# Many98/Crop2Seg

Hardware: AMD Instinct MI355X
Metric: train patches/sec (Tx10x128x128) U-TAE (higher is better)
Workload: dtype f32

## Files before the change

### crop2seg_amd/csrc/loss.hip

```cpp
#include "common.h"

namespace {

constexpr int MAXK = C2S_MAX_CLASSES;
constexpr int LOSS_BLOCKS = 512;

__device__ __forceinline__ bool valid_target(long long t, int K, long long ignore_index) {
    return !(t == ignore_index || t < 0 || t >= K);
}

__device__ __forceinline__ size_t pixel_offset(long e, int K, int HW) {
    const int pix = (int)(e % HW), b = (int)(e / HW);
    return (size_t)b * K * HW + pix;
}

__device__ __forceinline__ void zero_row(float* __restrict__ gp, int K, int HW) {
    for (int k = 0; k < K; ++k) gp[(size_t)k * HW] = 0.f;
}

template <bool FAST>
__device__ __forceinline__ void softmax_stats(const float* __restrict__ lp, int K, int HW, float& mx, float& s) {
    mx = lp[0];
    for (int k = 1; k < K; ++k) mx = fmaxf(mx, lp[(size_t)k * HW]);
    s = 0.f;
    for (int k = 0; k < K; ++k) s += FAST ? __expf(lp[(size_t)k * HW] - mx) : expf(lp[(size_t)k * HW] - mx);
}

template <int N>
__device__ __forceinline__ void block_partials(float (&v)[N], float* __restrict__ part) {
    __shared__ float red[4][N];
#pragma unroll
    for (int j = 0; j < N; ++j) v[j] = wave_sum(v[j]);
    if ((threadIdx.x & 63) == 0)
        for (int j = 0; j < N; ++j) red[threadIdx.x >> 6][j] = v[j];
    __syncthreads();
    if (threadIdx.x == 0)
        for (int j = 0; j < N; ++j) part[blockIdx.x * N + j] = (red[0][j] + red[1][j]) + (red[2][j] + red[3][j]);
}

template <int N>
__device__ __forceinline__ void sum_partials(const float* __restrict__ part, int blocks, double (&acc)[N]) {
    for (int i = 0; i < blocks; ++i) {
#pragma unroll
        for (int j = 0; j < N; ++j) acc[j] += part[i * N + j];
    }
}
__device__ __forceinline__ void store_loss(float* __restrict__ loss, float l, int accumulate) {
    *loss = accumulate ? *loss + l : l;
}

__global__ __launch_bounds__(256) void ce_fwd_kernel(const float* __restrict__ logits, const int64_t* __restrict__ target,
                                                     const float* __restrict__ cw, float* __restrict__ part, int B, int K,
                                                     int HW, float eps, long long ignore_index) {
    const long total = (long)B * HW;
    float num = 0.f, den = 0.f, bad = 0.f;
    for (long e = blockIdx.x * (long)blockDim.x + threadIdx.x; e < total; e += (long)gridDim.x * blockDim.x) {
        const long long yy = target[e];
        if (!valid_target(yy, K, ignore_index)) { bad += yy != ignore_index ? 1.f : 0.f; continue; }
        const int y = (int)yy;
        const float* lp = logits + pixel_offset(e, K, HW);
        float mx, s;
        softmax_stats<true>(lp, K, HW, mx, s);
        const float w = cw[y];
        const float lse = mx + __logf(s);
        float li = w * (lse - lp[(size_t)y * HW]);
        if (eps > 0.f) {
            float sm = 0.f;
            for (int k = 0; k < K; ++k) sm += cw[k] * (lse - lp[(size_t)k * HW]);
            li = (1.f - eps) * li + (eps / (float)K) * sm;
        }
        num += li;
        den += w;
    }
    float v[3] = {num, den, bad};
    block_partials(v, part);
}

__global__ void ce_finalize_kernel(const float* __restrict__ part, float* __restrict__ tot, float* __restrict__ loss,
                                   int blocks) {
    if (threadIdx.x != 0 || blockIdx.x != 0) return;
    double a[3] = {};
    sum_partials(part, blocks, a);
    tot[0] = (float)a[0]; tot[1] = (float)a[1]; tot[2] = (float)a[2];
    store_loss(loss, (float)(a[0] / a[1]), 0);
}

__global__ __launch_bounds__(256) void ce_bwd_kernel(const float* __restrict__ logits, const int64_t* __restrict__ target,
                                                     const float* __restrict__ cw, const float* __restrict__ tot,
                                                     float* __restrict__ glogits, int B, int K, int HW, float eps,
                                                     long long ignore_index) {
    const long total = (long)B * HW;
    const float inv_den = 1.f / tot[1];
    float wsum = 0.f;
    if (eps > 0.f)
        for (int k = 0; k < K; ++k) wsum += cw[k];
    for (long e = blockIdx.x * (long)blockDim.x + threadIdx.x; e < total; e += (long)gridDim.x * blockDim.x) {
        const float* lp = logits + pixel_offset(e, K, HW);
        float* gp = glogits + pixel_offset(e, K, HW);
        const long long yy = target[e];
        if (!valid_target(yy, K, ignore_index)) { zero_row(gp, K, HW); continue; }
        const int y = (int)yy;
        float mx, s;
        softmax_stats<true>(lp, K, HW, mx, s);
        const float w = cw[y] * inv_den, inv_s = 1.f / s;
        if (eps > 0.f) {
            const float a = (1.f - eps) * w, c = eps / (float)K * inv_den;
            for (int k = 0; k < K; ++k) {
                const float pk = __expf(lp[(size_t)k * HW] - mx) * inv_s;
                gp[(size_t)k * HW] = a * (pk - (k == y ? 1.f : 0.f)) + c * (wsum * pk - cw[k]);
            }
        } else {
            for (int k = 0; k < K; ++k)
                gp[(size_t)k * HW] = w * (__expf(lp[(size_t)k * HW] - mx) * inv_s - (k == y ? 1.f : 0.f));
        }
    }
}

__global__ __launch_bounds__(256) void focal_fwd_kernel(const float* __restrict__ logits, const int64_t* __restrict__ target,
                                                        const float* __restrict__ class_w, float* __restrict__ part, int B, int K,
                                                        int HW, float gamma, long long ignore_index) {
    const long total = (long)B * HW;
    float num = 0.f, cnt = 0.f, wsum = 0.f;
    for (long e = blockIdx.x * 256L + threadIdx.x; e < total; e += (long)gridDim.x * 256) {
        const long long t = target[e];
        if (!valid_target(t, K, ignore_index)) continue;
        const float* lp = logits + pixel_offset(e, K, HW);
        float mx, s;
        softmax_stats<false>(lp, K, HW, mx, s);
        const float logpt = lp[(size_t)t * HW] - mx - logf(s);
        const float pt = expf(logpt);
        num += -powf(1.f - pt, gamma) * logpt;
        cnt += 1.f;
        wsum += class_w ? class_w[t] : 1.f;
    }
    float v[3] = {num, cnt, wsum};
    block_partials(v, part);
}

__global__ void focal_finalize_kernel(const float* __restrict__ part, float* __restrict__ tot, float* __restrict__ loss,
                                      int blocks, int weighted, int size_average, int accumulate) {
    if (threadIdx.x != 0 || blockIdx.x != 0) return;
    double a[3] = {};
    sum_partials(part, blocks, a);
    const double num = a[0], cnt = a[1], wsum = a[2];
    const double scale = weighted ? (size_average ? wsum / (cnt * cnt) : wsum) : (size_average ? 1.0 / cnt : 1.0);
    tot[0] = (float)num; tot[1] = (float)cnt; tot[2] = (float)scale;
    store_loss(loss, (float)(num * scale), accumulate);
}

__global__ __launch_bounds__(256) void focal_bwd_kernel(const float* __restrict__ logits, const int64_t* __restrict__ target,
                                                        const float* __restrict__ tot, float* __restrict__ glogits, int B,
                                                        int K, int HW, float gamma, long long ignore_index) {
    const long total = (long)B * HW;
    const float inv_n = tot[2];
    for (long e = blockIdx.x * 256L + threadIdx.x; e < total; e += (long)gridDim.x * 256) {
        const float* lp = logits + pixel_offset(e, K, HW);
        float* gp = glogits + pixel_offset(e, K, HW);
        const long long t = target[e];
        if (!valid_target(t, K, ignore_index)) { zero_row(gp, K, HW); continue; }
        float mx, s;
        softmax_stats<false>(lp, K, HW, mx, s);
        const float inv_s = 1.f / s;
        const float logpt = lp[(size_t)t * HW] - mx - logf(s);
        const float pt = expf(logpt);
        const float om = 1.f - pt;
        const bool at_limit = gamma < 1.f && (gamma == 0.f || om <= 0.f);
        const float om_gm1 = at_limit ? 0.f : powf(om, gamma - 1.f);
        const float coef = (gamma * om_gm1 * pt * logpt - powf(om, gamma)) * inv_n;
        for (int k = 0; k < K; ++k) {
            const float pk = expf(lp[(size_t)k * HW] - mx) * inv_s;
            gp[(size_t)k * HW] = coef * ((k == t ? 1.f : 0.f) - pk);
        }
    }
}

__global__ __launch_bounds__(256) void smooth_ce_kernel(const float* __restrict__ logits, const int64_t* __restrict__ target,
// ... 21 lines not shown
        if (r < H - 1) { const long long v = target[e + W]; if (v >= 0 && v < K) mask |= 1u << (int)v; }
        if (x > 0) { const long long v = target[e - 1]; if (v >= 0 && v < K) mask |= 1u << (int)v; }
        if (x < W - 1) { const long long v = target[e + 1]; if (v >= 0 && v < K) mask |= 1u << (int)v; }
        const float nd = (float)__popc(mask);
        const float exp_small = eps * ((float)K - nd);
        const float exp_large = (1.f - exp_small) / nd;
        const bool is_bg = bg != nullptr && t == bg_index;
        float mx, s;
        softmax_stats<false>(lp, K, HW, mx, s);
        const float lse = mx + logf(s);
        const float inv_s = 1.f / s;
        float loss = 0.f, wsum = 0.f;
        for (int k = 0; k < K; ++k) {
            const float tk = is_bg ? bg[k] : (((mask >> k) & 1u) ? exp_large : eps);
            const float wt = (class_w ? class_w[k] : 1.f) * tk;
            loss -= wt * (lp[(size_t)k * HW] - lse);
            wsum += wt;
        }
        num += loss;
        if (pixel_loss) pixel_loss[e] = loss;
        if (gp) {
            for (int k = 0; k < K; ++k) {
                const float tk = is_bg ? bg[k] : (((mask >> k) & 1u) ? exp_large : eps);
                const float wt = (class_w ? class_w[k] : 1.f) * tk;
                const float pk = expf(lp[(size_t)k * HW] - mx) * inv_s;
                gp[(size_t)k * HW] = (pk * wsum - wt) * inv_n;
            }
        }
    }
    float v[2] = {num, bad};
    block_partials(v, part);
}

__global__ void smooth_ce_finalize_kernel(const float* __restrict__ part, float* __restrict__ tot, float* __restrict__ loss,
                                          int blocks, double npix, int accumulate) {
    if (threadIdx.x != 0 || blockIdx.x != 0) return;
    double a[2] = {};
    sum_partials(part, blocks, a);
    tot[0] = (float)a[0]; tot[1] = (float)a[1];
    store_loss(loss, (float)(a[0] / npix), accumulate);
}

constexpr int NCOUNT = 2 * MAXK + 1;

inline size_t recall_ws_floats(long n) { return (size_t)n + LOSS_BLOCKS + (2 * NCOUNT + 1) + MAXK + 2; }

__global__ void recall_zero_kernel(unsigned long long* __restrict__ cnt) {
    for (int i = threadIdx.x; i < NCOUNT; i += blockDim.x) cnt[i] = 0ull;
}

__device__ __forceinline__ void load_pixel(const float* __restrict__ lp, int K, int HW, float (&v)[MAXK]) {
#pragma unroll
    for (int k = 0; k < MAXK; ++k)
        if (k < K) v[k] = lp[(size_t)k * HW];
}

__global__ __launch_bounds__(256) void recall_count_kernel(const float* __restrict__ logits, const int64_t* __restrict__ target,
                                                           float* __restrict__ nll, unsigned long long* __restrict__ cnt, int B,
                                                           int K, int HW, long long ignore_index) {
    __shared__ unsigned int h[NCOUNT];
    for (int i = threadIdx.x; i < NCOUNT; i += 256) h[i] = 0;
    __syncthreads();
    const long total = (long)B * HW;
    for (long e = blockIdx.x * 256L + threadIdx.x; e < total; e += (long)gridDim.x * 256) {
        const long long t = target[e];
        if (!valid_target(t, K, ignore_index)) {
            if (t != ignore_index) atomicAdd(&h[2 * MAXK], 1u);
            nll[e] = 0.f;
            continue;
        }
        float v[MAXK];
// ... 19 lines not shown
    for (int i = threadIdx.x; i < NCOUNT; i += 256)
        if (h[i]) atomicAdd(cnt + i, (unsigned long long)h[i]);
}

__global__ void recall_weights_kernel(const unsigned long long* __restrict__ cnt, float* __restrict__ w, float* __restrict__ tot,
                                      float* __restrict__ weights_out, long long* __restrict__ counts_out, int K) {
    const int k = threadIdx.x;
    if (k < K) {
        const unsigned long long gt = cnt[k], fn = cnt[MAXK + k];
        const float wk = (float)((double)(fn > 0 ? fn : 1ull) / (double)(gt > 0 ? gt : 1ull));
        w[k] = wk;
        if (weights_out) weights_out[k] = wk;
        if (counts_out) { counts_out[k] = (long long)gt; counts_out[K + k] = (long long)fn; }
    }
    if (k == 0) tot[1] = (float)cnt[2 * MAXK];
}

__global__ __launch_bounds__(256) void recall_loss_kernel(const float* __restrict__ nll, const int64_t* __restrict__ target,
                                                          const float* __restrict__ w, float* __restrict__ part, long total,
                                                          int K, long long ignore_index) {
    __shared__ float ws[MAXK];
    if (threadIdx.x < K) ws[threadIdx.x] = w[threadIdx.x];
    __syncthreads();
    float num = 0.f;
    for (long e = blockIdx.x * 256L + threadIdx.x; e < total; e += (long)gridDim.x * 256) {
        const long long t = target[e];
        if (!valid_target(t, K, ignore_index)) continue;
        num += ws[(int)t] * nll[e];
    }
    float v[1] = {num};
    block_partials(v, part);
}

__global__ void recall_finalize_kernel(const float* __restrict__ part, float* __restrict__ tot, float* __restrict__ loss,
                                       int blocks, double npix, int accumulate) {
    if (threadIdx.x != 0 || blockIdx.x != 0) return;
    double a[1] = {};
    sum_partials(part, blocks, a);
    tot[0] = (float)a[0];
    store_loss(loss, (float)(a[0] / npix), accumulate);
}

__global__ __launch_bounds__(256) void recall_bwd_kernel(const float* __restrict__ logits, const int64_t* __restrict__ target,
                                                         const float* __restrict__ w, float* __restrict__ glogits, int B, int K,
                                                         int HW, long long ignore_index, float inv_n) {
    __shared__ float ws[MAXK];
    if (threadIdx.x < K) ws[threadIdx.x] = w[threadIdx.x];
    __syncthreads();
    const long total = (long)B * HW;
    for (long e = blockIdx.x * 256L + threadIdx.x; e < total; e += (long)gridDim.x * 256) {
        float* gp = glogits + pixel_offset(e, K, HW);
        const long long t = target[e];
        if (!valid_target(t, K, ignore_index)) { zero_row(gp, K, HW); continue; }
        float v[MAXK];
        load_pixel(logits + pixel_offset(e, K, HW), K, HW, v);
        float mx = v[0];
#pragma unroll
        for (int k = 1; k < MAXK; ++k)
            if (k < K) mx = fmaxf(mx, v[k]);
        float s = 0.f;
#pragma unroll
        for (int k = 0; k < MAXK; ++k)
            if (k < K) { v[k] = expf(v[k] - mx); s += v[k]; }
        const float inv_s = 1.f / s, c = ws[(int)t] * inv_n;
#pragma unroll
        for (int k = 0; k < MAXK; ++k)
            if (k < K) gp[(size_t)k * HW] = c * (v[k] * inv_s - (k == (int)t ? 1.f : 0.f));
    }
}

}

extern "C" size_t c2s_cross_entropy_workspace_floats(int, int) { return 3 * LOSS_BLOCKS + 3; }

extern "C" int c2s_cross_entropy(const float* logits, const int64_t* target, const float* class_w, float* loss,
                                 float* glogits, int B, int K, int HW, float label_smoothing, long long ignore_index,
                                 float* workspace, size_t ws_floats, void* stream) {
    C2S_REQUIRE(logits && target && class_w && loss && workspace, "cross_entropy: null pointer");
    C2S_REQUIRE(ws_floats >= 3 * LOSS_BLOCKS + 3 && B > 0 && K > 0 && HW > 0, "cross_entropy: bad args");
    C2S_REQUIRE(label_smoothing >= 0.f && label_smoothing <= 1.f, "cross_entropy: label_smoothing must be in [0, 1]");
    hipStream_t st = (hipStream_t)stream;
    const int blocks = grid_for((long)B * HW, LOSS_BLOCKS);
    float* tot = workspace + 3 * LOSS_BLOCKS;
    hipLaunchKernelGGL(ce_fwd_kernel, dim3(blocks), dim3(256), 0, st, logits, target, class_w, workspace, B, K, HW,
                       label_smoothing, ignore_index);
    C2S_CHECK_LAUNCH("ce_fwd");
    hipLaunchKernelGGL(ce_finalize_kernel, dim3(1), dim3(64), 0, st, workspace, tot, loss, blocks);
    C2S_CHECK_LAUNCH("ce_finalize");
    if (glogits != nullptr) {
        hipLaunchKernelGGL(ce_bwd_kernel, dim3(blocks), dim3(256), 0, st, logits, target, class_w, tot, glogits, B, K, HW,
                           label_smoothing, ignore_index);
        C2S_CHECK_LAUNCH("ce_bwd");
    }
    return C2S_OK;
}

extern "C" size_t c2s_focal_ce_workspace_floats(void) { return 3 * LOSS_BLOCKS + 4; }

extern "C" int c2s_focal_ce_ex(const float* logits, const long long* target, const float* class_w, float* loss, float* glogits,
                               int B, int K, int HW, float gamma, long long ignore_index, int size_average, int accumulate_loss,
                               float* workspace, size_t ws_floats, void* stream) {
    C2S_REQUIRE(logits && target && loss && workspace, "focal_ce: null pointer");
    C2S_REQUIRE(B > 0 && K > 0 && HW > 0 && gamma >= 0.f, "focal_ce: bad args");
    C2S_REQUIRE(ws_floats >= c2s_focal_ce_workspace_floats(), "focal_ce: workspace too small");
    hipStream_t st = (hipStream_t)stream;
    const int blocks = grid_for((long)B * HW, LOSS_BLOCKS);
    float* tot = workspace + 3 * LOSS_BLOCKS;
    hipLaunchKernelGGL(focal_fwd_kernel, dim3(blocks), dim3(256), 0, st, logits, (const int64_t*)target, class_w, workspace, B, K,
                       HW, gamma, ignore_index);
    C2S_CHECK_LAUNCH("focal_fwd");
    hipLaunchKernelGGL(focal_finalize_kernel, dim3(1), dim3(64), 0, st, workspace, tot, loss, blocks, class_w != nullptr ? 1 : 0,
                       size_average, accumulate_loss);
    C2S_CHECK_LAUNCH("focal_finalize");
    if (glogits) {
        hipLaunchKernelGGL(focal_bwd_kernel, dim3(grid_for((long)B * HW, 2048)), dim3(256), 0, st, logits, (const int64_t*)target, tot,
                           glogits, B, K, HW, gamma, ignore_index);
        C2S_CHECK_LAUNCH("focal_bwd");
    }
    return C2S_OK;
}

extern "C" int c2s_focal_ce(const float* logits, const long long* target, float* loss, float* glogits, int B, int K, int HW,
                            float gamma, long long ignore_index, int accumulate_loss, float* workspace, size_t ws_floats,
                            void* stream) {
    return c2s_focal_ce_ex(logits, target, nullptr, loss, glogits, B, K, HW, gamma, ignore_index, 1, accumulate_loss, workspace,
                           ws_floats, stream);
}

extern "C" size_t c2s_smooth_ce_workspace_floats(void) { return 2 * LOSS_BLOCKS + 2; }

extern "C" int c2s_smooth_ce_ex(const float* logits, const long long* target, const float* class_w, const float* bg_distrib,
                                float* loss, float* glogits, float* pixel_loss, int B, int K, int H, int W, float label_smoothing,
                                long long bg_index, int reduction, int accumulate_loss, float* workspace, size_t ws_floats,
                                void* stream) {
    C2S_REQUIRE(logits && target && loss && workspace, "smooth_ce: null pointer");
    C2S_REQUIRE(B > 0 && H > 0 && W > 0 && K >= 1 && K <= MAXK, "smooth_ce: 1 <= K <= 32 classes");
    C2S_REQUIRE(label_smoothing >= 0.f && label_smoothing <= 1.f, "smooth_ce: label_smoothing outside [0, 1]");
    C2S_REQUIRE(reduction >= 0 && reduction <= 2 && (reduction != 2 || pixel_loss != nullptr), "smooth_ce: reduction 0 mean / 1 sum / 2 none (needs pixel_loss)");
    C2S_REQUIRE(ws_floats >= c2s_smooth_ce_workspace_floats(), "smooth_ce: workspace too small");
    hipStream_t st = (hipStream_t)stream;
    const int blocks = grid_for((long)B * H * W, LOSS_BLOCKS);
    float* tot = workspace + 2 * LOSS_BLOCKS;
    const double npix = reduction == 0 ? (double)B * H * W : 1.0;
    hipLaunchKernelGGL(smooth_ce_kernel, dim3(blocks), dim3(256), 0, st, logits, (const int64_t*)target, class_w, bg_distrib,
                       workspace, glogits, pixel_loss, B, K, H, W, label_smoothing, bg_index, (float)(1.0 / npix));
    C2S_CHECK_LAUNCH("smooth_ce");
    hipLaunchKernelGGL(smooth_ce_finalize_kernel, dim3(1), dim3(64), 0, st, workspace, tot, loss, blocks, npix, accumulate_loss);
    C2S_CHECK_LAUNCH("smooth_ce_finalize");
    return C2S_OK;
}

extern "C" int c2s_smooth_ce(const float* logits, const long long* target, const float* class_w, const float* bg_distrib,
                             float* loss, float* glogits, int B, int K, int H, int W, float label_smoothing,
                             long long bg_index, int accumulate_loss, float* workspace, size_t ws_floats, void* stream) {
    return c2s_smooth_ce_ex(logits, target, class_w, bg_distrib, loss, glogits, nullptr, B, K, H, W, label_smoothing, bg_index, 0,
                            accumulate_loss, workspace, ws_floats, stream);
}

extern "C" size_t c2s_recall_ce_workspace_floats(int B, int HW) {
    return (B > 0 && HW > 0) ? recall_ws_floats((long)B * HW) : recall_ws_floats(0);
}

extern "C" int c2s_recall_ce(const float* logits, const long long* target, float* loss, float* glogits, float* weights_out,
                             long long* counts_out, int B, int K, int HW, long long ignore_index, int accumulate_loss,
                             float* workspace, size_t ws_floats, void* stream) {
    C2S_REQUIRE(K >= 1 && K <= MAXK, "recall_ce: 1 <= K <= 32 classes (got %d)", K);
    C2S_REQUIRE(logits && target && loss && workspace, "recall_ce: null pointer");
    C2S_REQUIRE(B > 0 && HW > 0, "recall_ce: bad args");
    C2S_REQUIRE(ws_floats >= c2s_recall_ce_workspace_floats(B, HW), "recall_ce: workspace too small");
    hipStream_t st = (hipStream_t)stream;
    const long n = (long)B * HW;
    const int blocks = grid_for(n, LOSS_BLOCKS);
    float* nll = workspace;
    float* part = workspace + n;
    float* cnt_f = part + LOSS_BLOCKS;
    if (((uintptr_t)cnt_f & 7) != 0) ++cnt_f;
    unsigned long long* cnt = (unsigned long long*)cnt_f;
    float* w = part + LOSS_BLOCKS + (2 * NCOUNT + 1);
    float* tot = w + MAXK;
    hipLaunchKernelGGL(recall_zero_kernel, dim3(1), dim3(128), 0, st, cnt);
    C2S_CHECK_LAUNCH("recall_zero");
    hipLaunchKernelGGL(recall_count_kernel, dim3(blocks), dim3(256), 0, st, logits, (const int64_t*)target, nll, cnt, B, K, HW,
                       ignore_index);
    C2S_CHECK_LAUNCH("recall_count");
    hipLaunchKernelGGL(recall_weights_kernel, dim3(1), dim3(64), 0, st, cnt, w, tot, weights_out, counts_out, K);
    C2S_CHECK_LAUNCH("recall_weights");
    hipLaunchKernelGGL(recall_loss_kernel, dim3(blocks), dim3(256), 0, st, nll, (const int64_t*)target, w, part, n, K,
                       ignore_index);
    C2S_CHECK_LAUNCH("recall_loss");
    hipLaunchKernelGGL(recall_finalize_kernel, dim3(1), dim3(64), 0, st, part, tot, loss, blocks, (double)n, accumulate_loss);
    C2S_CHECK_LAUNCH("recall_finalize");
    if (glogits != nullptr) {
        hipLaunchKernelGGL(recall_bwd_kernel, dim3(blocks), dim3(256), 0, st, logits, (const int64_t*)target, w, glogits, B, K, HW,
                           ignore_index, (float)(1.0 / (double)n));
        C2S_CHECK_LAUNCH("recall_bwd");
    }
    return C2S_OK;
}
```

### crop2seg_amd/csrc/ltae.hip

```cpp
#include "common.h"
#include "ltae_drop.h"
#include "ltae_long.h"

#define C2S_AS1 __attribute__((address_space(1)))
#define C2S_AS3 __attribute__((address_space(3)))

namespace {

#ifdef C2S_LT_STAMP
__device__ unsigned long long lt_stamps[4096 * 8];
__device__ unsigned long long lt_stamps_bwd[4096 * 8];
#define LT_STAMP(k) do { if (threadIdx.x == 0 && blockIdx.x < 4096) lt_stamps[blockIdx.x * 8 + (k)] = __builtin_amdgcn_s_memtime(); } while (0)
#define LT_STAMP_B(k) do { if (threadIdx.x == 0 && blockIdx.x < 4096) lt_stamps_bwd[blockIdx.x * 8 + (k)] = __builtin_amdgcn_s_memtime(); } while (0)
#else
#define LT_STAMP(k)
#define LT_STAMP_B(k)
#endif

constexpr int NH = 16;
constexpr int DV = 16;

struct LtaeParams {
    const float* x; const float* gamma; const float* beta; const float* U; const float* s0;
    const float* Wc; const float* bc; const float* pe; const int* valid;
// ... 936 lines not shown
        __syncthreads();
        if constexpr (GX) {
            m1 = group_total(m1, red) * inv_n;
            m2 = group_total(m2, red + 256) * inv_n;
        }
        const float dgs = (dg.x + dg.y) + (dg.z + dg.w), dbs = (db.x + db.y) + (db.z + db.w);
        if constexpr (NTH > 1) {
            red[512 + (sth * C + sc_) * 2] = dgs;
            red[512 + (sth * C + sc_) * 2 + 1] = dbs;
            __syncthreads();
            if (sth == 0) {
                float a = 0.f, bsum = 0.f;
#pragma unroll
                for (int k = 0; k < NTH; ++k) { a += red[512 + (k * C + sc_) * 2]; bsum += red[512 + (k * C + sc_) * 2 + 1]; }
                p.part_gb[((size_t)tile * C + sc_) * 2] = a;
                p.part_gb[((size_t)tile * C + sc_) * 2 + 1] = bsum;
            }
        } else {
            p.part_gb[((size_t)tile * C + sc_) * 2] = dgs;
            p.part_gb[((size_t)tile * C + sc_) * 2 + 1] = dbs;
        }
        if constexpr (!GX) return;
        const f32x4 rstd = *reinterpret_cast<const f32x4*>(STl + g * 8 + 4);
        for (int t = sth; t < T; t += NTH) {
            f32x4* gp = reinterpret_cast<f32x4*>(gxc + (size_t)t * C * HW);
            const f32x4 xn = *reinterpret_cast<const f32x4*>(xs + (size_t)(t * CP + sc_) * 4);
            *gp = rstd * (*gp - m1 - xn * m2);
        }
    }
}

constexpr int RR_SLICES = 32;
template <typename TI, typename TO>
__global__ __launch_bounds__(1024) void reduce_rows_kernel(const TI* __restrict__ part, TO* __restrict__ out, TO* __restrict__ out1,
                                                           int count, int K, int slices, int rows_per_slice) {
    __shared__ double sh[16][64];
    const int lane = threadIdx.x & 63, w = threadIdx.x >> 6;
    const int k = blockIdx.x * 64 + lane;
    const int grp = blockIdx.y / slices, sl = blockIdx.y - grp * slices;
    const int r0 = sl * rows_per_slice;
    const int n = count - r0 < rows_per_slice ? count - r0 : rows_per_slice;
    const bool live = k < K;
    const TI* src = part + ((size_t)grp * count + r0) * K + (live ? k : 0);
    double s = 0.0;
    for (int i0 = w; i0 < n; i0 += 256) {
        TI v[16];
#pragma unroll
        for (int u = 0; u < 16; ++u) {
            const int i = i0 + 16 * u;
            v[u] = (live && i < n) ? src[(size_t)i * K] : TI(0);
        }
#pragma unroll
        for (int u = 0; u < 16; ++u) s += (double)v[u];
    }
    sh[w][lane] = s;
    __syncthreads();
    if (w == 0 && live) {
        double t = 0.0;
#pragma unroll
        for (int ww = 0; ww < 16; ++ww) t += sh[ww][lane];
        if (out1 != nullptr) ((k & 1) ? out1 : out)[k >> 1] = (TO)t;
        else out[(size_t)blockIdx.y * K + k] = (TO)t;
    }
}

void reduce_rows(const float* part, float* out, int groups, int count, int K, double* tmp, hipStream_t st, float* out1 = nullptr) {
    const int kb = (K + 63) / 64;
    if (count <= 512 || tmp == nullptr) {
        hipLaunchKernelGGL((reduce_rows_kernel<float, float>), dim3(kb, groups), dim3(1024), 0, st, part, out, out1, count, K, 1, count);
    } else {
        const int rps_min = (count + RR_SLICES - 1) / RR_SLICES;
        const int rps = rps_min > 256 ? rps_min : 256;
        const int slices = (count + rps - 1) / rps;
        hipLaunchKernelGGL((reduce_rows_kernel<float, double>), dim3(kb, groups * slices), dim3(1024), 0, st, part, tmp, (double*)nullptr,
                           count, K, slices, rps);
        hipLaunchKernelGGL((reduce_rows_kernel<double, float>), dim3(kb, groups), dim3(1024), 0, st, (const double*)tmp, out, out1,
                           slices, K, 1, slices);
    }
}

__global__ __launch_bounds__(64) void sum_over_pixels_kernel(const float* __restrict__ V, float* __restrict__ out, int B,
                                                             int rows, int HW) {
    const int row = blockIdx.x, lane = threadIdx.x;
    float s = 0.f;
    for (int b = 0; b < B; ++b) {
        const float* v = V + ((size_t)b * rows + row) * HW;
        for (int i = lane; i < HW; i += 64) s += v[i];
    }
    s = wave_sum(s);
    if (lane == 0) out[row] = s;
}

template <int NH = 16, int DV = 16>
__global__ __launch_bounds__(256) void gwc_kernel(const float* __restrict__ ge, const float* __restrict__ Z,
                                                  float* __restrict__ gWc, int B, int C, int HW) {
    const int h = blockIdx.x / C, c = blockIdx.x % C;
    const int q = threadIdx.x & 15;
#pragma unroll
    for (int j0 = 0; j0 < DV; j0 += 16) {
        const int j = j0 + (threadIdx.x >> 4);
        if (DV < 16 && j >= DV) break;
        float s = 0.f;
        for (int b = 0; b < B; ++b) {
            const float* z = Z + (((size_t)b * NH + h) * C + c) * HW;
            const float* g = ge + ((size_t)b * NH * DV + h * DV + j) * HW;
            for (int i = q; i < HW; i += 16) s += g[i] * z[i];
        }
        s += __shfl_xor(s, 1, 64); s += __shfl_xor(s, 2, 64); s += __shfl_xor(s, 4, 64); s += __shfl_xor(s, 8, 64);
        if (q == 0) gWc[(size_t)(h * DV + j) * C + c] = s;
    }
}

typedef float f32x4v __attribute__((ext_vector_type(4)));
constexpr int GW_PITCH = 68;
__global__ __launch_bounds__(256) void gwc_mfma_kernel(const float* __restrict__ ge, const float* __restrict__ Z,
                                                       float* __restrict__ part, int B, int HW, int tiles_per_slice) {
    constexpr int C = 64;
    __shared__ float tl[(DV + C) * GW_PITCH];
    const int h = blockIdx.x, slice = blockIdx.y;
    const int tid = threadIdx.x, lane = tid & 63, w = tid >> 6;
    const int tiles_per_b = HW / 64;
    const int ntiles = B * tiles_per_b;
    f32x4v acc = {0.f, 0.f, 0.f, 0.f};
    for (int tile = slice * tiles_per_slice; tile < (slice + 1) * tiles_per_slice && tile < ntiles; ++tile) {
        const int b = tile / tiles_per_b, pix0 = (tile % tiles_per_b) * 64;
        __syncthreads();
#pragma unroll
        for (int i = 0; i < 5; ++i) {
            const int e = tid + i * 256;
            const int row = e >> 4, q = e & 15;
            const float* src = row < DV ? ge + ((size_t)b * NH * DV + h * DV + row) * HW
                                        : Z + (((size_t)b * NH + h) * C + (row - DV)) * HW;
            *reinterpret_cast<f32x4v*>(tl + row * GW_PITCH + 4 * q) = *reinterpret_cast<const f32x4v*>(src + pix0 + 4 * q);
        }
        __syncthreads();
        const float* ap = tl + (lane & 15) * GW_PITCH + (lane >> 4);
        const float* bp = tl + (DV + w * 16 + (lane & 15)) * GW_PITCH + (lane >> 4);
#pragma unroll
        for (int ks = 0; ks < 16; ++ks) acc = __builtin_amdgcn_mfma_f32_16x16x4f32(ap[4 * ks], bp[4 * ks], acc, 0, 0, 0);
// ... 140 lines not shown
    }
    acc = wave_sum(acc);
    if (lane == 0) {
        const float vb = rsq * qv * S;
        gbk[hd] = acc_bk ? gbk[hd] + vb : vb;
        const float vq = rsq * (acc + bk[hd] * S);
        gQ[hd] = acc_q ? gQ[hd] + vq : vq;
    }
}

__global__ void pixel_gn_fwd_kernel(const float* __restrict__ x, const float* __restrict__ gamma,
                                    const float* __restrict__ beta, float* __restrict__ y, float* __restrict__ stats,
                                    int B, int C, int HW, int groups, float eps) {
    const long total = (long)B * groups * HW;
    const long e = blockIdx.x * (long)blockDim.x + threadIdx.x;
    if (e >= total) return;
    const int pix = (int)(e % HW);
    const long bg = e / HW;
    const int g = (int)(bg % groups), b = (int)(bg / groups);
    const int cpg = C / groups;
    const float* xp = x + ((size_t)b * C + g * cpg) * HW + pix;
    float s = 0.f;
    for (int c = 0; c < cpg; ++c) s += xp[(size_t)c * HW];
    const float mean = s / cpg;
    float m2 = 0.f;
    for (int c = 0; c < cpg; ++c) { const float d = xp[(size_t)c * HW] - mean; m2 += d * d; }
    const float rstd = rsqrtf(m2 / cpg + eps);
    stats[e * 2] = mean; stats[e * 2 + 1] = rstd;
    float* yp = y + ((size_t)b * C + g * cpg) * HW + pix;
    for (int c = 0; c < cpg; ++c)
        yp[(size_t)c * HW] = (xp[(size_t)c * HW] - mean) * rstd * gamma[g * cpg + c] + beta[g * cpg + c];
}

__global__ __launch_bounds__(64) void pixel_gn_bwd_kernel(const float* __restrict__ x, const float* __restrict__ gy,
                                                          const float* __restrict__ gamma, const float* __restrict__ stats,
                                                          float* __restrict__ gx, float* __restrict__ part, int B, int C,
                                                          int HW, int groups, int chunks) {
    const int lane = threadIdx.x;
    const int chunk = blockIdx.x % chunks;
    const int bg = blockIdx.x / chunks;
    const int g = bg % groups, b = bg / groups;
    const int cpg = C / groups;
    const int len = (HW + chunks - 1) / chunks;
    const int beg = chunk * len, end = (beg + len) < HW ? (beg + len) : HW;
    float dg[16], db[16];
#pragma unroll
    for (int c = 0; c < 16; ++c) { dg[c] = 0.f; db[c] = 0.f; }
    for (int pix = beg + lane; pix < end; pix += 64) {
        const long e = ((long)b * groups + g) * HW + pix;
        const float mean = stats[e * 2], rstd = stats[e * 2 + 1];
        const float* xp = x + ((size_t)b * C + g * cpg) * HW + pix;
        const float* gp = gy + ((size_t)b * C + g * cpg) * HW + pix;
        float m1 = 0.f, m2 = 0.f;
#pragma unroll
        for (int c = 0; c < 16; ++c)
            if (c < cpg) {
                const float xn = (xp[(size_t)c * HW] - mean) * rstd;
                const float gg = gp[(size_t)c * HW];
                dg[c] += gg * xn; db[c] += gg;
                const float dxn = gg * gamma[g * cpg + c];
                m1 += dxn; m2 += dxn * xn;
            }
        m1 /= cpg; m2 /= cpg;
        float* gxp = gx + ((size_t)b * C + g * cpg) * HW + pix;
#pragma unroll
        for (int c = 0; c < 16; ++c)
            if (c < cpg) {
                const float xn = (xp[(size_t)c * HW] - mean) * rstd;
                gxp[(size_t)c * HW] = rstd * (gp[(size_t)c * HW] * gamma[g * cpg + c] - m1 - xn * m2);
            }
    }
#pragma unroll
    for (int c = 0; c < 16; ++c)
        if (c < cpg) {
            const float a = wave_sum(dg[c]), bb = wave_sum(db[c]);
            if (lane == 0) {
                const size_t o = (((size_t)b * chunks + chunk) * C + g * cpg + c) * 2;
                part[o] = a; part[o + 1] = bb;
            }
        }
}

__global__ void dropout_nchw_kernel(const float* __restrict__ x, float* __restrict__ y, int B, int C, int HW, float p,
                                    uint64_t seed0, const uint64_t* __restrict__ seed_dev, const float* __restrict__ keep) {
    const uint64_t seed = seed0 + (seed_dev != nullptr ? *seed_dev * 0x9E3779B97F4A7C15ull : 0ull);
    const long total = (long)B * C * HW;
    const float inv = 1.f / (1.f - p);
    for (long e = blockIdx.x * (long)blockDim.x + threadIdx.x; e < total; e += (long)gridDim.x * blockDim.x) {
        const int pix = (int)(e % HW);
        const long bc = e / HW;
        const int c = (int)(bc % C), b = (int)(bc / C);
        const long idx = ((long)b * HW + pix) * C + c;
        const bool k = keep != nullptr ? keep[idx] != 0.f : c2s_uniform(seed, (uint64_t)idx) >= p;
        y[e] = k ? x[e] * inv : 0.f;
    }
}

__global__ void ltae_prep_kernel(const float* __restrict__ U, const float* __restrict__ gamma, const float* __restrict__ beta,
                                 float* __restrict__ Ut, float* __restrict__ cU, int C) {
    const int tid = threadIdx.x;
    for (int e = tid; e < C * NH; e += blockDim.x) {
        const int c = e / NH, h = e % NH;
        Ut[e] = U[h * C + c] * gamma[c];
    }
    if (tid < NH) {
        float s = 0.f;
        for (int c = 0; c < C; ++c) s = fmaf(U[tid * C + c], beta[c], s);
        cU[tid] = s;
    }
}


template <int CPG>
// ... 2083 lines not shown
            else hipLaunchKernelGGL((ltae_lds_bwd_kernel<256, false>), tiles, dim3(256), lb, st, p, sb);
        }
        C2S_CHECK_LAUNCH("ltae_lds_bwd");
        break;
    }
    case BWD_TILE8:
        launch_tile_bwd_heads(d, p, tiles, st);
        C2S_CHECK_LAUNCH("ltae_bwd_heads");
        break;
    }
    switch (pl.dx) {
    case DX_GX64: {
        const dim3 grid(d->B * (d->HW / 64));
        if (gx != nullptr) hipLaunchKernelGGL(ltae_stream_bwd_gx64_kernel<true>, grid, dim3(1024), GX_FLOATS * sizeof(float) + 8192, st, p, sb);
        else hipLaunchKernelGGL(ltae_stream_bwd_gx64_kernel<false>, grid, dim3(1024), GX_FLOATS * sizeof(float) + 8192, st, p, sb);
        C2S_CHECK_LAUNCH("ltae_stream_bwd_gx");
        break;
    }
    case DX_GX4: {
        const size_t lds2 = ((size_t)NH * d->C * SPT + 2 * SCH * 4 * SPT * 4) * sizeof(float);
        hipLaunchKernelGGL(ltae_stream_bwd_gx_kernel<4>, tiles, dim3(1024), lds2, st, p, sb);
        C2S_CHECK_LAUNCH("ltae_stream_bwd_gx");
        break;
    }
    case DX_TILE8:
        if (gx != nullptr) launch_tile_bwd_gx<true>(d, p, tiles, st);
        else launch_tile_bwd_gx<false>(d, p, tiles, st);
        C2S_CHECK_LAUNCH("ltae_bwd_gx");
        break;
    case DX_NONE: case DX_FUSED:
        break;
    }
    const int nh = d->n_head, dm = d->d_model;
    reduce_rows(p.part_s0, gs0, d->B, (d->HW + pl.px - 1) / pl.px, d->T * nh, rtmp, st);
    C2S_CHECK_LAUNCH("ltae_reduce_s0");
    reduce_rows(p.part_bc, gbc, 1, (int)pl.tiles, dm, rtmp, st);
    C2S_CHECK_LAUNCH("ltae_reduce_bc");
    if (call.gb) {
        reduce_rows(p.part_gb, ggamma, 1, pl.gb_tiles, 2 * d->C, rtmp, st, gbeta);
        C2S_CHECK_LAUNCH("ltae_reduce_gb");
    }
    if (pl.gU_rows) reduce_rows(part_U, gU, 1, (int)pl.tiles, nh * d->C, rtmp, st);
    else hipLaunchKernelGGL(sum_over_pixels_kernel, dim3(nh * d->C), dim3(64), 0, st, p.V, gU, d->B, nh * d->C, d->HW);
    C2S_CHECK_LAUNCH("ltae_gU");
    switch (pl.gwc) {
    case GWC_MFMA: {
        float* part_wc = workspace + ws.part_wc;
        const int tps = (d->B * (d->HW / 64) + pl.wc_slices - 1) / pl.wc_slices;
        hipLaunchKernelGGL(gwc_mfma_kernel, dim3(NH, pl.wc_slices), dim3(256), 0, st, g_emb, p.Z, part_wc, d->B, d->HW, tps);
        C2S_CHECK_LAUNCH("ltae_gWc_mfma");
        reduce_rows(part_wc, gWc, 1, pl.wc_slices, NH * DV * d->C, nullptr, st);
        C2S_CHECK_LAUNCH("ltae_gWc_reduce");
        break;
    }
    case GWC_DIRECT: {
#define F(H, D) hipLaunchKernelGGL((gwc_kernel<H, D>), dim3(nh * d->C), dim3(256), 0, st, g_emb, p.Z, gWc, d->B, d->C, d->HW)
        C2S_LTAE_HEADS(d, F)
#undef F
        C2S_CHECK_LAUNCH("ltae_gWc");
        break;
    }
    case GWC_ZERO:
        hipMemsetAsync(gWc, 0, (size_t)dm * d->C * sizeof(float), st);
        break;
    }
    return C2S_OK;
}

extern "C" int c2s_positional_table_ex(const long long* dates, float* pe, long n, float period, int d_v, void* stream) {
    C2S_REQUIRE(dates && pe && n > 0 && period > 0.f && d_v > 0, "positional_table: bad args");
    hipLaunchKernelGGL(positional_table_kernel, dim3(cdiv(n * d_v, 256)), dim3(256), 0, (hipStream_t)stream, dates, pe, n, period, d_v);
    C2S_CHECK_LAUNCH("positional_table");
    return C2S_OK;
}

extern "C" int c2s_positional_table(const long long* dates, float* pe, long n, float period, void* stream) {
    return c2s_positional_table_ex(dates, pe, n, period, DV, stream);
// ... 72 lines not shown

extern "C" int c2s_ltae_fold_bwd(const float* Q, const float* Wk, const float* bk, const float* Wc, const float* bc,
                                 const float* pe, const float* qwk, const float* gU, const float* gs0,
                                 const float* gWc_attn, const float* gbc_attn, float* gQ, float* gWk, float* gbk,
                                 float* gWc, float* gbc, int BT, int C, int acc_mask, float* workspace, size_t ws_floats,
                                 void* stream) {
    return c2s_ltae_fold_bwd_ex(Q, Wk, bk, Wc, bc, pe, qwk, gU, gs0, gWc_attn, gbc_attn, gQ, gWk, gbk, gWc, gbc, BT, C, NH, 4,
                                NH * DV, acc_mask, workspace, ws_floats, stream);
}

extern "C" int c2s_pixel_gn_fwd(const float* x, const float* gamma, const float* beta, float* y, float* stats, int B,
                                int C, int HW, int groups, float eps, void* stream) {
    C2S_REQUIRE(x && gamma && beta && y && stats && groups > 0 && C % groups == 0 && C / groups <= 16, "pixel_gn_fwd: bad args");
    const long total = (long)B * groups * HW;
    hipLaunchKernelGGL(pixel_gn_fwd_kernel, dim3(cdiv(total, 256)), dim3(256), 0, (hipStream_t)stream, x, gamma, beta, y,
                       stats, B, C, HW, groups, eps);
    C2S_CHECK_LAUNCH("pixel_gn_fwd");
    return C2S_OK;
}

extern "C" size_t c2s_pixel_gn_bwd_workspace_floats(int B, int C, int HW) {
    const int chunks = cdiv(HW, 256);
    return (size_t)B * chunks * C * 2 + 2 * (size_t)C;
}

extern "C" int c2s_pixel_gn_bwd(const float* x, const float* gy, const float* gamma, const float* stats, float* gx,
                                float* dgamma, float* dbeta, int B, int C, int HW, int groups, float* workspace,
                                size_t ws_floats, void* stream) {
    C2S_REQUIRE(x && gy && gamma && stats && gx && dgamma && dbeta && workspace, "pixel_gn_bwd: null pointer");
    C2S_REQUIRE(groups > 0 && C % groups == 0 && C / groups <= 16, "pixel_gn_bwd: bad groups");
    C2S_REQUIRE(ws_floats >= c2s_pixel_gn_bwd_workspace_floats(B, C, HW), "pixel_gn_bwd: workspace too small");
    const int chunks = cdiv(HW, 256);
    hipStream_t st = (hipStream_t)stream;
    hipLaunchKernelGGL(pixel_gn_bwd_kernel, dim3(B * groups * chunks), dim3(64), 0, st, x, gy, gamma, stats, gx, workspace,
                       B, C, HW, groups, chunks);
    C2S_CHECK_LAUNCH("pixel_gn_bwd");
    reduce_rows(workspace, dgamma, 1, B * chunks, 2 * C, nullptr, st, dbeta);
    C2S_CHECK_LAUNCH("pixel_gn_reduce");
    return C2S_OK;
}

extern "C" int c2s_dropout_nchw(const float* x, float* y, int B, int C, int HW, float p, uint64_t seed,
                                const uint64_t* seed_dev, const float* keep,
                                void* stream) {
    C2S_REQUIRE(x && y && p >= 0.f && p < 1.f, "dropout: bad args");
    const long total = (long)B * C * HW;
    const int blocks = (int)((total + 255) / 256 > 4096 ? 4096 : (total + 255) / 256);
    hipLaunchKernelGGL(dropout_nchw_kernel, dim3(blocks), dim3(256), 0, (hipStream_t)stream, x, y, B, C, HW, p, seed, seed_dev, keep);
    C2S_CHECK_LAUNCH("dropout");
    return C2S_OK;
}
```

Measured before the change: 385.2.

## Fuse loss finalize into backward, batch L-TAE reductions, widen GN backward and gWc

```diff
diff --git a/crop2seg_amd/csrc/loss.hip b/crop2seg_amd/csrc/loss.hip
--- a/crop2seg_amd/csrc/loss.hip
+++ b/crop2seg_amd/csrc/loss.hip
@@ -40,10 +40,23 @@
 
 template <int N>
 __device__ __forceinline__ void sum_partials(const float* __restrict__ part, int blocks, double (&acc)[N]) {
-    for (int i = 0; i < blocks; ++i) {
+    __shared__ double tot_red[4][N];
+#pragma unroll
+    for (int j = 0; j < N; ++j) acc[j] = 0.0;
+    for (int i = threadIdx.x; i < blocks; i += 256) {
 #pragma unroll
         for (int j = 0; j < N; ++j) acc[j] += part[i * N + j];
     }
+#pragma unroll
+    for (int j = 0; j < N; ++j) {
+#pragma unroll
+        for (int o = 32; o > 0; o >>= 1) acc[j] += __shfl_xor(acc[j], o, 64);
+    }
+    if ((threadIdx.x & 63) == 0)
+        for (int j = 0; j < N; ++j) tot_red[threadIdx.x >> 6][j] = acc[j];
+    __syncthreads();
+#pragma unroll
+    for (int j = 0; j < N; ++j) acc[j] = (tot_red[0][j] + tot_red[1][j]) + (tot_red[2][j] + tot_red[3][j]);
 }
 __device__ __forceinline__ void store_loss(float* __restrict__ loss, float l, int accumulate) {
     *loss = accumulate ? *loss + l : l;
@@ -76,21 +89,29 @@
     block_partials(v, part);
 }
 
-__global__ void ce_finalize_kernel(const float* __restrict__ part, float* __restrict__ tot, float* __restrict__ loss,
-                                   int blocks) {
-    if (threadIdx.x != 0 || blockIdx.x != 0) return;
-    double a[3] = {};
+__device__ __forceinline__ float ce_totals(const float* __restrict__ part, int blocks, float* __restrict__ tot,
+                                           float* __restrict__ loss) {
+    double a[3];
     sum_partials(part, blocks, a);
-    tot[0] = (float)a[0]; tot[1] = (float)a[1]; tot[2] = (float)a[2];
-    store_loss(loss, (float)(a[0] / a[1]), 0);
+    if (blockIdx.x == 0 && threadIdx.x == 0) {
+        tot[0] = (float)a[0]; tot[1] = (float)a[1]; tot[2] = (float)a[2];
+        store_loss(loss, (float)(a[0] / a[1]), 0);
+    }
+    return (float)a[1];
+}
+
+__global__ __launch_bounds__(256) void ce_finalize_kernel(const float* __restrict__ part, float* __restrict__ tot,
+                                                          float* __restrict__ loss, int blocks) {
+    ce_totals(part, blocks, tot, loss);
 }
 
 __global__ __launch_bounds__(256) void ce_bwd_kernel(const float* __restrict__ logits, const int64_t* __restrict__ target,
-                                                     const float* __restrict__ cw, const float* __restrict__ tot,
+                                                     const float* __restrict__ cw, const float* __restrict__ part,
+                                                     float* __restrict__ tot, float* __restrict__ loss,
                                                      float* __restrict__ glogits, int B, int K, int HW, float eps,
                                                      long long ignore_index) {
     const long total = (long)B * HW;
-    const float inv_den = 1.f / tot[1];
+    const float inv_den = 1.f / ce_totals(part, (int)gridDim.x, tot, loss);
     float wsum = 0.f;
     if (eps > 0.f)
         for (int k = 0; k < K; ++k) wsum += cw[k];
@@ -137,11 +158,12 @@
     block_partials(v, part);
 }
 
-__global__ void focal_finalize_kernel(const float* __restrict__ part, float* __restrict__ tot, float* __restrict__ loss,
-                                      int blocks, int weighted, int size_average, int accumulate) {
-    if (threadIdx.x != 0 || blockIdx.x != 0) return;
-    double a[3] = {};
+__global__ __launch_bounds__(256) void focal_finalize_kernel(const float* __restrict__ part, float* __restrict__ tot,
+                                                             float* __restrict__ loss, int blocks, int weighted,
+                                                             int size_average, int accumulate) {
+    double a[3];
     sum_partials(part, blocks, a);
+    if (threadIdx.x != 0) return;
     const double num = a[0], cnt = a[1], wsum = a[2];
     const double scale = weighted ? (size_average ? wsum / (cnt * cnt) : wsum) : (size_average ? 1.0 / cnt : 1.0);
     tot[0] = (float)num; tot[1] = (float)cnt; tot[2] = (float)scale;
@@ -229,11 +251,12 @@
     block_partials(v, part);
 }
 
-__global__ void smooth_ce_finalize_kernel(const float* __restrict__ part, float* __restrict__ tot, float* __restrict__ loss,
-                                          int blocks, double npix, int accumulate) {
-    if (threadIdx.x != 0 || blockIdx.x != 0) return;
-    double a[2] = {};
+__global__ __launch_bounds__(256) void smooth_ce_finalize_kernel(const float* __restrict__ part, float* __restrict__ tot,
+                                                                 float* __restrict__ loss, int blocks, double npix,
+                                                                 int accumulate) {
+    double a[2];
     sum_partials(part, blocks, a);
+    if (threadIdx.x != 0) return;
     tot[0] = (float)a[0]; tot[1] = (float)a[1];
     store_loss(loss, (float)(a[0] / npix), accumulate);
 }
@@ -319,11 +342,12 @@
     block_partials(v, part);
 }
 
-__global__ void recall_finalize_kernel(const float* __restrict__ part, float* __restrict__ tot, float* __restrict__ loss,
-                                       int blocks, double npix, int accumulate) {
-    if (threadIdx.x != 0 || blockIdx.x != 0) return;
-    double a[1] = {};
+__global__ __launch_bounds__(256) void recall_finalize_kernel(const float* __restrict__ part, float* __restrict__ tot,
+                                                              float* __restrict__ loss, int blocks, double npix,
+                                                              int accumulate) {
+    double a[1];
     sum_partials(part, blocks, a);
+    if (threadIdx.x != 0) return;
     tot[0] = (float)a[0];
     store_loss(loss, (float)(a[0] / npix), accumulate);
 }
@@ -372,12 +396,13 @@
     hipLaunchKernelGGL(ce_fwd_kernel, dim3(blocks), dim3(256), 0, st, logits, target, class_w, workspace, B, K, HW,
                        label_smoothing, ignore_index);
     C2S_CHECK_LAUNCH("ce_fwd");
-    hipLaunchKernelGGL(ce_finalize_kernel, dim3(1), dim3(64), 0, st, workspace, tot, loss, blocks);
-    C2S_CHECK_LAUNCH("ce_finalize");
     if (glogits != nullptr) {
-        hipLaunchKernelGGL(ce_bwd_kernel, dim3(blocks), dim3(256), 0, st, logits, target, class_w, tot, glogits, B, K, HW,
-                           label_smoothing, ignore_index);
+        hipLaunchKernelGGL(ce_bwd_kernel, dim3(blocks), dim3(256), 0, st, logits, target, class_w, workspace, tot, loss, glogits, B,
+                           K, HW, label_smoothing, ignore_index);
         C2S_CHECK_LAUNCH("ce_bwd");
+    } else {
+        hipLaunchKernelGGL(ce_finalize_kernel, dim3(1), dim3(256), 0, st, workspace, tot, loss, blocks);
+        C2S_CHECK_LAUNCH("ce_finalize");
     }
     return C2S_OK;
 }
@@ -396,7 +421,7 @@
     hipLaunchKernelGGL(focal_fwd_kernel, dim3(blocks), dim3(256), 0, st, logits, (const int64_t*)target, class_w, workspace, B, K,
                        HW, gamma, ignore_index);
     C2S_CHECK_LAUNCH("focal_fwd");
-    hipLaunchKernelGGL(focal_finalize_kernel, dim3(1), dim3(64), 0, st, workspace, tot, loss, blocks, class_w != nullptr ? 1 : 0,
+    hipLaunchKernelGGL(focal_finalize_kernel, dim3(1), dim3(256), 0, st, workspace, tot, loss, blocks, class_w != nullptr ? 1 : 0,
                        size_average, accumulate_loss);
     C2S_CHECK_LAUNCH("focal_finalize");
     if (glogits) {
@@ -432,7 +457,7 @@
     hipLaunchKernelGGL(smooth_ce_kernel, dim3(blocks), dim3(256), 0, st, logits, (const int64_t*)target, class_w, bg_distrib,
                        workspace, glogits, pixel_loss, B, K, H, W, label_smoothing, bg_index, (float)(1.0 / npix));
     C2S_CHECK_LAUNCH("smooth_ce");
-    hipLaunchKernelGGL(smooth_ce_finalize_kernel, dim3(1), dim3(64), 0, st, workspace, tot, loss, blocks, npix, accumulate_loss);
+    hipLaunchKernelGGL(smooth_ce_finalize_kernel, dim3(1), dim3(256), 0, st, workspace, tot, loss, blocks, npix, accumulate_loss);
     C2S_CHECK_LAUNCH("smooth_ce_finalize");
     return C2S_OK;
 }
@@ -475,7 +500,7 @@
     hipLaunchKernelGGL(recall_loss_kernel, dim3(blocks), dim3(256), 0, st, nll, (const int64_t*)target, w, part, n, K,
                        ignore_index);
     C2S_CHECK_LAUNCH("recall_loss");
-    hipLaunchKernelGGL(recall_finalize_kernel, dim3(1), dim3(64), 0, st, part, tot, loss, blocks, (double)n, accumulate_loss);
+    hipLaunchKernelGGL(recall_finalize_kernel, dim3(1), dim3(256), 0, st, part, tot, loss, blocks, (double)n, accumulate_loss);
     C2S_CHECK_LAUNCH("recall_finalize");
     if (glogits != nullptr) {
         hipLaunchKernelGGL(recall_bwd_kernel, dim3(blocks), dim3(256), 0, st, logits, (const int64_t*)target, w, glogits, B, K, HW,
diff --git a/crop2seg_amd/csrc/ltae.hip b/crop2seg_amd/csrc/ltae.hip
--- a/crop2seg_amd/csrc/ltae.hip
+++ b/crop2seg_amd/csrc/ltae.hip
@@ -992,12 +992,12 @@
 
 constexpr int RR_SLICES = 32;
 template <typename TI, typename TO>
-__global__ __launch_bounds__(1024) void reduce_rows_kernel(const TI* __restrict__ part, TO* __restrict__ out, TO* __restrict__ out1,
-                                                           int count, int K, int slices, int rows_per_slice) {
+__device__ __forceinline__ void reduce_rows_block(const TI* __restrict__ part, TO* __restrict__ out, TO* __restrict__ out1,
+                                                  int count, int K, int slices, int rows_per_slice, int bx, int by) {
     __shared__ double sh[16][64];
     const int lane = threadIdx.x & 63, w = threadIdx.x >> 6;
-    const int k = blockIdx.x * 64 + lane;
-    const int grp = blockIdx.y / slices, sl = blockIdx.y - grp * slices;
+    const int k = bx * 64 + lane;
+    const int grp = by / slices, sl = by - grp * slices;
     const int r0 = sl * rows_per_slice;
     const int n = count - r0 < rows_per_slice ? count - r0 : rows_per_slice;
     const bool live = k < K;
@@ -1020,8 +1020,24 @@
 #pragma unroll
         for (int ww = 0; ww < 16; ++ww) t += sh[ww][lane];
         if (out1 != nullptr) ((k & 1) ? out1 : out)[k >> 1] = (TO)t;
-        else out[(size_t)blockIdx.y * K + k] = (TO)t;
-    }
+        else out[(size_t)by * K + k] = (TO)t;
+    }
+}
+template <typename TI, typename TO>
+__global__ __launch_bounds__(1024) void reduce_rows_kernel(const TI* __restrict__ part, TO* __restrict__ out, TO* __restrict__ out1,
+                                                           int count, int K, int slices, int rows_per_slice) {
+    reduce_rows_block(part, out, out1, count, K, slices, rows_per_slice, (int)blockIdx.x, (int)blockIdx.y);
+}
+
+constexpr int RR_JOBS = 4;
+struct RRJob { const float* part; float* out; float* out1; int groups, count, K; };
+struct RRBatch { RRJob job[RR_JOBS]; int first[RR_JOBS + 1]; int n; };
+__global__ __launch_bounds__(1024) void reduce_rows_batch_kernel(RRBatch b) {
+    int j = 0;
+    while (j + 1 < b.n && (int)blockIdx.x >= b.first[j + 1]) ++j;
+    const RRJob& q = b.job[j];
+    const int local = (int)blockIdx.x - b.first[j], kb = (q.K + 63) / 64;
+    reduce_rows_block(q.part, q.out, q.out1, q.count, q.K, 1, q.count, local % kb, local / kb);
 }
 
 void reduce_rows(const float* part, float* out, int groups, int count, int K, double* tmp, hipStream_t st, float* out1 = nullptr) {
@@ -1038,6 +1054,22 @@
                            slices, K, 1, slices);
     }
 }
+void reduce_rows_batch(const RRJob* jobs, int n, double* tmp, hipStream_t st) {
+    bool one_pass = n > 1 && n <= RR_JOBS;
+    for (int j = 0; j < n; ++j) one_pass = one_pass && (jobs[j].count <= 512 || tmp == nullptr);
+    if (!one_pass) {
+        for (int j = 0; j < n; ++j)
+            reduce_rows(jobs[j].part, jobs[j].out, jobs[j].groups, jobs[j].count, jobs[j].K, tmp, st, jobs[j].out1);
+        return;
+    }
+    RRBatch b = {};
+    b.n = n;
+    for (int j = 0; j < n; ++j) {
+        b.job[j] = jobs[j];
+        b.first[j + 1] = b.first[j] + (jobs[j].K + 63) / 64 * jobs[j].groups;
+    }
+    hipLaunchKernelGGL(reduce_rows_batch_kernel, dim3(b.first[n]), dim3(1024), 0, st, b);
+}
 
 __global__ __launch_bounds__(64) void sum_over_pixels_kernel(const float* __restrict__ V, float* __restrict__ out, int B,
                                                              int rows, int HW) {
@@ -1051,6 +1083,7 @@
     if (lane == 0) out[row] = s;
 }
 
+constexpr int GW_UNROLL = 16;
 template <int NH = 16, int DV = 16>
 __global__ __launch_bounds__(256) void gwc_kernel(const float* __restrict__ ge, const float* __restrict__ Z,
                                                   float* __restrict__ gWc, int B, int C, int HW) {
@@ -1064,7 +1097,17 @@
         for (int b = 0; b < B; ++b) {
             const float* z = Z + (((size_t)b * NH + h) * C + c) * HW;
             const float* g = ge + ((size_t)b * NH * DV + h * DV + j) * HW;
-            for (int i = q; i < HW; i += 16) s += g[i] * z[i];
+            for (int i0 = q; i0 < HW; i0 += 16 * GW_UNROLL) {
+                float gv[GW_UNROLL], zv[GW_UNROLL];
+#pragma unroll
+                for (int u = 0; u < GW_UNROLL; ++u) {
+                    const int i = i0 + 16 * u < HW ? i0 + 16 * u : i0;
+                    gv[u] = g[i]; zv[u] = z[i];
+                }
+#pragma unroll
+                for (int u = 0; u < GW_UNROLL; ++u)
+                    if (i0 + 16 * u < HW) s = fmaf(gv[u], zv[u], s);
+            }
         }
         s += __shfl_xor(s, 1, 64); s += __shfl_xor(s, 2, 64); s += __shfl_xor(s, 4, 64); s += __shfl_xor(s, 8, 64);
         if (q == 0) gWc[(size_t)(h * DV + j) * C + c] = s;
@@ -1271,53 +1314,69 @@
         yp[(size_t)c * HW] = (xp[(size_t)c * HW] - mean) * rstd * gamma[g * cpg + c] + beta[g * cpg + c];
 }
 
-__global__ __launch_bounds__(64) void pixel_gn_bwd_kernel(const float* __restrict__ x, const float* __restrict__ gy,
-                                                          const float* __restrict__ gamma, const float* __restrict__ stats,
-                                                          float* __restrict__ gx, float* __restrict__ part, int B, int C,
-                                                          int HW, int groups, int chunks) {
-    const int lane = threadIdx.x;
+__global__ __launch_bounds__(256) void pixel_gn_bwd_kernel(const float* __restrict__ x, const float* __restrict__ gy,
+                                                           const float* __restrict__ gamma, const float* __restrict__ stats,
+                                                           float* __restrict__ gx, float* __restrict__ part, int B, int C,
+                                                           int HW, int groups, int chunks) {
+    __shared__ float chain[32][64];
+    const int lane = threadIdx.x & 63, w = threadIdx.x >> 6;
     const int chunk = blockIdx.x % chunks;
     const int bg = blockIdx.x / chunks;
     const int g = bg % groups, b = bg / groups;
     const int cpg = C / groups;
     const int len = (HW + chunks - 1) / chunks;
     const int beg = chunk * len, end = (beg + len) < HW ? (beg + len) : HW;
-    float dg[16], db[16];
-#pragma unroll
-    for (int c = 0; c < 16; ++c) { dg[c] = 0.f; db[c] = 0.f; }
-    for (int pix = beg + lane; pix < end; pix += 64) {
+    const int pix = beg + lane + 64 * w;
+    const bool live = pix < end;
+    float xn[16], gg[16];
+    if (live) {
         const long e = ((long)b * groups + g) * HW + pix;
-        const float mean = stats[e * 2], rstd = stats[e * 2 + 1];
-        const float* xp = x + ((size_t)b * C + g * cpg) * HW + pix;
-        const float* gp = gy + ((size_t)b * C + g * cpg) * HW + pix;
+        const float2 st = *reinterpret_cast<const float2*>(stats + e * 2);
+        const float mean = st.x, rstd = st.y;
+        const size_t o = ((size_t)b * C + g * cpg) * HW + pix;
+#pragma unroll
+        for (int c = 0; c < 16; ++c) {
+            const int cc = c < cpg ? c : cpg - 1;
+            xn[c] = x[o + (size_t)cc * HW];
+            gg[c] = gy[o + (size_t)cc * HW];
+        }
         float m1 = 0.f, m2 = 0.f;
 #pragma unroll
         for (int c = 0; c < 16; ++c)
             if (c < cpg) {
-                const float xn = (xp[(size_t)c * HW] - mean) * rstd;
-                const float gg = gp[(size_t)c * HW];
-                dg[c] += gg * xn; db[c] += gg;
-                const float dxn = gg * gamma[g * cpg + c];
-                m1 += dxn; m2 += dxn * xn;
+                xn[c] = __fmul_rn(__fsub_rn(xn[c], mean), rstd);
+                const float dxn = __fmul_rn(gg[c], gamma[g * cpg + c]);
+                m1 = __fadd_rn(m1, dxn);
+                m2 = __fadd_rn(m2, __fmul_rn(dxn, xn[c]));
             }
         m1 /= cpg; m2 /= cpg;
-        float* gxp = gx + ((size_t)b * C + g * cpg) * HW + pix;
 #pragma unroll
         for (int c = 0; c < 16; ++c)
             if (c < cpg) {
-                const float xn = (xp[(size_t)c * HW] - mean) * rstd;
-                gxp[(size_t)c * HW] = rstd * (gp[(size_t)c * HW] * gamma[g * cpg + c] - m1 - xn * m2);
-            }
-    }
-#pragma unroll
-    for (int c = 0; c < 16; ++c)
-        if (c < cpg) {
-            const float a = wave_sum(dg[c]), bb = wave_sum(db[c]);
-            if (lane == 0) {
-                const size_t o = (((size_t)b * chunks + chunk) * C + g * cpg + c) * 2;
-                part[o] = a; part[o + 1] = bb;
-            }
-        }
+                const float gm = gamma[g * cpg + c];
+                const float t = c < 15 ? fmaf(gg[c], gm, -m1) : __fsub_rn(__fmul_rn(gg[c], gm), m1);
+                gx[o + (size_t)c * HW] = __fmul_rn(rstd, fmaf(-m2, xn[c], t));
+            }
+    }
+    for (int k = 0; k < 4; ++k) {
+        if (w == k) {
+#pragma unroll
+            for (int c = 0; c < 16; ++c)
+                if (c < cpg) {
+                    float dg = k ? chain[c][lane] : 0.f, db = k ? chain[16 + c][lane] : 0.f;
+                    if (live) { dg = fmaf(gg[c], xn[c], dg); db = __fadd_rn(db, gg[c]); }
+                    chain[c][lane] = dg; chain[16 + c][lane] = db;
+                }
+        }
+        __syncthreads();
+    }
+    for (int c = w; c < cpg; c += 4) {
+        const float a = wave_sum(chain[c][lane]), bb = wave_sum(chain[16 + c][lane]);
+        if (lane == 0) {
+            const size_t o = (((size_t)b * chunks + chunk) * C + g * cpg + c) * 2;
+            part[o] = a; part[o + 1] = bb;
+        }
+    }
 }
 
 __global__ void dropout_nchw_kernel(const float* __restrict__ x, float* __restrict__ y, int B, int C, int HW, float p,
@@ -3467,17 +3526,18 @@
         break;
     }
     const int nh = d->n_head, dm = d->d_model;
-    reduce_rows(p.part_s0, gs0, d->B, (d->HW + pl.px - 1) / pl.px, d->T * nh, rtmp, st);
-    C2S_CHECK_LAUNCH("ltae_reduce_s0");
-    reduce_rows(p.part_bc, gbc, 1, (int)pl.tiles, dm, rtmp, st);
-    C2S_CHECK_LAUNCH("ltae_reduce_bc");
-    if (call.gb) {
-        reduce_rows(p.part_gb, ggamma, 1, pl.gb_tiles, 2 * d->C, rtmp, st, gbeta);
-        C2S_CHECK_LAUNCH("ltae_reduce_gb");
-    }
-    if (pl.gU_rows) reduce_rows(part_U, gU, 1, (int)pl.tiles, nh * d->C, rtmp, st);
-    else hipLaunchKernelGGL(sum_over_pixels_kernel, dim3(nh * d->C), dim3(64), 0, st, p.V, gU, d->B, nh * d->C, d->HW);
-    C2S_CHECK_LAUNCH("ltae_gU");
+    RRJob jobs[RR_JOBS];
+    int nj = 0;
+    jobs[nj++] = {p.part_s0, gs0, nullptr, d->B, (d->HW + pl.px - 1) / pl.px, d->T * nh};
+    jobs[nj++] = {p.part_bc, gbc, nullptr, 1, (int)pl.tiles, dm};
+    if (call.gb) jobs[nj++] = {p.part_gb, ggamma, gbeta, 1, pl.gb_tiles, 2 * d->C};
+    if (pl.gU_rows) jobs[nj++] = {part_U, gU, nullptr, 1, (int)pl.tiles, nh * d->C};
+    reduce_rows_batch(jobs, nj, rtmp, st);
+    C2S_CHECK_LAUNCH("ltae_reduce");
+    if (!pl.gU_rows) {
+        hipLaunchKernelGGL(sum_over_pixels_kernel, dim3(nh * d->C), dim3(64), 0, st, p.V, gU, d->B, nh * d->C, d->HW);
+        C2S_CHECK_LAUNCH("ltae_gU");
+    }
     switch (pl.gwc) {
     case GWC_MFMA: {
         float* part_wc = workspace + ws.part_wc;
@@ -3616,7 +3676,7 @@
     C2S_REQUIRE(ws_floats >= c2s_pixel_gn_bwd_workspace_floats(B, C, HW), "pixel_gn_bwd: workspace too small");
     const int chunks = cdiv(HW, 256);
     hipStream_t st = (hipStream_t)stream;
-    hipLaunchKernelGGL(pixel_gn_bwd_kernel, dim3(B * groups * chunks), dim3(64), 0, st, x, gy, gamma, stats, gx, workspace,
+    hipLaunchKernelGGL(pixel_gn_bwd_kernel, dim3(B * groups * chunks), dim3(256), 0, st, x, gy, gamma, stats, gx, workspace,
                        B, C, HW, groups, chunks);
     C2S_CHECK_LAUNCH("pixel_gn_bwd");
     reduce_rows(workspace, dgamma, 1, B * chunks, 2 * C, nullptr, st, dbeta);
```

Measured after the change: 388.2, median of 6. Within noise of the previous version (+0.8%).
